# debbiemarkslab/EVcouplings

Hardware: NVIDIA H100
Metric: PLM gradient evals/s as N*L^2*q cell-ops/s (higher is better)
Workload: dtype f32 parameters/accumulation; tensor-core products as bf16 hi+lo pairs (16 mantissa bits)

## Files before the change

evcouplings_b200/csrc/plm_tc.cu:

```cuda
#include <cuda.h>
#include <cuda_bf16.h>

#include <stdlib.h>

#include <algorithm>

#include "common.cuh"
#include "internal.h"

namespace evc {

constexpr int TC_BM = 128;
constexpr int TC_BN = 192;
constexpr int TC_BK = 64;
constexpr int TC_MAX_STAGES = 8;
constexpr int TC_A_BYTES = TC_BM * TC_BK * 2;
constexpr int TC_B_BYTES = TC_BN * TC_BK * 2;
constexpr int TC_SMEM_LIMIT = 232448;
constexpr int TC_SMEM_HEAD = 2048;
constexpr int TC_THREADS = 384;
constexpr int TC_CONSUMERS = 256;
constexpr int TC_K_CHUNK = 32;
constexpr int TC_MAX_KSPLIT = 8;
constexpr int TC_REG_PRODUCER = 40;
constexpr int TC_REG_CONSUMER = 232;

__device__ __forceinline__ void mbar_wait_bounded(uint64_t *bar, uint32_t parity)
{
    uint32_t done = 0;
    for (uint64_t it = 0; it < (1ull << 31); it++) {
        asm volatile(
            "{\n.reg .pred p;\n"
            "mbarrier.try_wait.parity.shared::cta.b64 p, [%1], %2;\n"
            "selp.u32 %0, 1, 0, p;\n}\n"
            : "=r"(done)
            : "r"(smem_u32(bar)), "r"(parity)
            : "memory");
        if (done) return;
    }
    __trap();
}

__device__ __forceinline__ void mbar_arrive(uint64_t *bar)
{
    asm volatile("mbarrier.arrive.shared::cta.b64 _, [%0];" ::"r"(smem_u32(bar)) : "memory");
}

__device__ __forceinline__ void tma_load_2d(void *smem_dst, const CUtensorMap *tmap, int c0, int c1, uint64_t *bar)
{
    asm volatile(
        "cp.async.bulk.tensor.2d.shared::cluster.global.mbarrier::complete_tx::bytes [%0], [%1, {%3, %4}], [%2];"
        ::"r"(smem_u32(smem_dst)), "l"(reinterpret_cast<uint64_t>(tmap)), "r"(smem_u32(bar)), "r"(c0), "r"(c1)
        : "memory");
}

__device__ __forceinline__ void tma_load_2d_hint(void *smem_dst, const CUtensorMap *tmap, int c0, int c1,
                                                 uint64_t *bar, uint64_t policy)
{
    asm volatile(
        "cp.async.bulk.tensor.2d.shared::cluster.global.mbarrier::complete_tx::bytes.L2::cache_hint "
        "[%0], [%1, {%3, %4}], [%2], %5;"
        ::"r"(smem_u32(smem_dst)), "l"(reinterpret_cast<uint64_t>(tmap)), "r"(smem_u32(bar)), "r"(c0), "r"(c1),
        "l"(policy)
        : "memory");
}
__device__ __forceinline__ uint64_t l2_policy_evict_last()
{
    uint64_t p;
    asm volatile("createpolicy.fractional.L2::evict_last.b64 %0, 1.0;" : "=l"(p));
    return p;
}

template <int N>
__device__ __forceinline__ void setmaxnreg_dec() { asm volatile("setmaxnreg.dec.sync.aligned.u32 %0;\n" ::"n"(N)); }
template <int N>
__device__ __forceinline__ void setmaxnreg_inc() { asm volatile("setmaxnreg.inc.sync.aligned.u32 %0;\n" ::"n"(N)); }

__device__ __forceinline__ void wgmma_fence() { asm volatile("wgmma.fence.sync.aligned;" ::: "memory"); }
__device__ __forceinline__ void wgmma_commit() { asm volatile("wgmma.commit_group.sync.aligned;" ::: "memory"); }
template <int N>
__device__ __forceinline__ void wgmma_wait() { asm volatile("wgmma.wait_group.sync.aligned %0;" ::"n"(N) : "memory"); }

template <int R>
__device__ __forceinline__ void fence_regs(float *d)
{
#pragma unroll
    for (int i = 0; i < R; i++) asm volatile("" : "+f"(d[i])::"memory");
}

__device__ __forceinline__ void consumer_sync() { asm volatile("bar.sync 1, %0;" ::"n"(TC_CONSUMERS) : "memory"); }

__device__ __forceinline__ uint64_t make_desc_sw128(const void *smem_ptr)
{
    const uint32_t addr = smem_u32(smem_ptr);
    uint64_t d = 0;
    d |= (uint64_t)((addr >> 4) & 0x3FFF);
    d |= (uint64_t)1 << 16;
    d |= (uint64_t)(1024 >> 4) << 32;
    d |= (uint64_t)1 << 62;
    return d;
}

template <int N>
__device__ __forceinline__ void wgmma_bf16(float *d, uint64_t da, uint64_t db, uint32_t scale_d);
template <>
__device__ __forceinline__ void wgmma_bf16<192>(float *d, uint64_t da, uint64_t db, uint32_t scale_d)
{
    asm volatile(
        "{\n.reg .pred p;\n"
        "setp.ne.b32 p, %98, 0;\n"
        "wgmma.mma_async.sync.aligned.m64n192k16.f32.bf16.bf16 "
        "{"
        "%0, %1, %2, %3, %4, %5, %6, %7, %8, %9, %10, %11, %12, %13, %14, %15, "
        "%16, %17, %18, %19, %20, %21, %22, %23, %24, %25, %26, %27, %28, %29, %30, %31, "
        "%32, %33, %34, %35, %36, %37, %38, %39, %40, %41, %42, %43, %44, %45, %46, %47, "
        "%48, %49, %50, %51, %52, %53, %54, %55, %56, %57, %58, %59, %60, %61, %62, %63, "
        "%64, %65, %66, %67, %68, %69, %70, %71, %72, %73, %74, %75, %76, %77, %78, %79, "
        "%80, %81, %82, %83, %84, %85, %86, %87, %88, %89, %90, %91, %92, %93, %94, %95"
        "}, %96, %97, p, 1, 1, 0, 0;\n}\n"
        : "+f"(d[0]), "+f"(d[1]), "+f"(d[2]), "+f"(d[3]), "+f"(d[4]), "+f"(d[5]), "+f"(d[6]), "+f"(d[7]),
          "+f"(d[8]), "+f"(d[9]), "+f"(d[10]), "+f"(d[11]), "+f"(d[12]), "+f"(d[13]), "+f"(d[14]), "+f"(d[15]),
          "+f"(d[16]), "+f"(d[17]), "+f"(d[18]), "+f"(d[19]), "+f"(d[20]), "+f"(d[21]), "+f"(d[22]), "+f"(d[23]),
          "+f"(d[24]), "+f"(d[25]), "+f"(d[26]), "+f"(d[27]), "+f"(d[28]), "+f"(d[29]), "+f"(d[30]), "+f"(d[31]),
          "+f"(d[32]), "+f"(d[33]), "+f"(d[34]), "+f"(d[35]), "+f"(d[36]), "+f"(d[37]), "+f"(d[38]), "+f"(d[39]),
          "+f"(d[40]), "+f"(d[41]), "+f"(d[42]), "+f"(d[43]), "+f"(d[44]), "+f"(d[45]), "+f"(d[46]), "+f"(d[47]),
          "+f"(d[48]), "+f"(d[49]), "+f"(d[50]), "+f"(d[51]), "+f"(d[52]), "+f"(d[53]), "+f"(d[54]), "+f"(d[55]),
          "+f"(d[56]), "+f"(d[57]), "+f"(d[58]), "+f"(d[59]), "+f"(d[60]), "+f"(d[61]), "+f"(d[62]), "+f"(d[63]),
          "+f"(d[64]), "+f"(d[65]), "+f"(d[66]), "+f"(d[67]), "+f"(d[68]), "+f"(d[69]), "+f"(d[70]), "+f"(d[71]),
          "+f"(d[72]), "+f"(d[73]), "+f"(d[74]), "+f"(d[75]), "+f"(d[76]), "+f"(d[77]), "+f"(d[78]), "+f"(d[79]),
          "+f"(d[80]), "+f"(d[81]), "+f"(d[82]), "+f"(d[83]), "+f"(d[84]), "+f"(d[85]), "+f"(d[86]), "+f"(d[87]),
          "+f"(d[88]), "+f"(d[89]), "+f"(d[90]), "+f"(d[91]), "+f"(d[92]), "+f"(d[93]), "+f"(d[94]), "+f"(d[95])
        : "l"(da), "l"(db), "r"(scale_d));
}
template <>
__device__ __forceinline__ void wgmma_bf16<176>(float *d, uint64_t da, uint64_t db, uint32_t scale_d)
{
    asm volatile(
        "{\n.reg .pred p;\n"
        "setp.ne.b32 p, %90, 0;\n"
        "wgmma.mma_async.sync.aligned.m64n176k16.f32.bf16.bf16 "
        "{"
        "%0, %1, %2, %3, %4, %5, %6, %7, %8, %9, %10, %11, %12, %13, %14, %15, "
        "%16, %17, %18, %19, %20, %21, %22, %23, %24, %25, %26, %27, %28, %29, %30, %31, "
        "%32, %33, %34, %35, %36, %37, %38, %39, %40, %41, %42, %43, %44, %45, %46, %47, "
        "%48, %49, %50, %51, %52, %53, %54, %55, %56, %57, %58, %59, %60, %61, %62, %63, "
        "%64, %65, %66, %67, %68, %69, %70, %71, %72, %73, %74, %75, %76, %77, %78, %79, "
        "%80, %81, %82, %83, %84, %85, %86, %87"
        "}, %88, %89, p, 1, 1, 0, 0;\n}\n"
        : "+f"(d[0]), "+f"(d[1]), "+f"(d[2]), "+f"(d[3]), "+f"(d[4]), "+f"(d[5]), "+f"(d[6]), "+f"(d[7]),
          "+f"(d[8]), "+f"(d[9]), "+f"(d[10]), "+f"(d[11]), "+f"(d[12]), "+f"(d[13]), "+f"(d[14]), "+f"(d[15]),
          "+f"(d[16]), "+f"(d[17]), "+f"(d[18]), "+f"(d[19]), "+f"(d[20]), "+f"(d[21]), "+f"(d[22]), "+f"(d[23]),
          "+f"(d[24]), "+f"(d[25]), "+f"(d[26]), "+f"(d[27]), "+f"(d[28]), "+f"(d[29]), "+f"(d[30]), "+f"(d[31]),
          "+f"(d[32]), "+f"(d[33]), "+f"(d[34]), "+f"(d[35]), "+f"(d[36]), "+f"(d[37]), "+f"(d[38]), "+f"(d[39]),
          "+f"(d[40]), "+f"(d[41]), "+f"(d[42]), "+f"(d[43]), "+f"(d[44]), "+f"(d[45]), "+f"(d[46]), "+f"(d[47]),
          "+f"(d[48]), "+f"(d[49]), "+f"(d[50]), "+f"(d[51]), "+f"(d[52]), "+f"(d[53]), "+f"(d[54]), "+f"(d[55]),
          "+f"(d[56]), "+f"(d[57]), "+f"(d[58]), "+f"(d[59]), "+f"(d[60]), "+f"(d[61]), "+f"(d[62]), "+f"(d[63]),
          "+f"(d[64]), "+f"(d[65]), "+f"(d[66]), "+f"(d[67]), "+f"(d[68]), "+f"(d[69]), "+f"(d[70]), "+f"(d[71]),
          "+f"(d[72]), "+f"(d[73]), "+f"(d[74]), "+f"(d[75]), "+f"(d[76]), "+f"(d[77]), "+f"(d[78]), "+f"(d[79]),
          "+f"(d[80]), "+f"(d[81]), "+f"(d[82]), "+f"(d[83]), "+f"(d[84]), "+f"(d[85]), "+f"(d[86]), "+f"(d[87])
        : "l"(da), "l"(db), "r"(scale_d));
}

template <int N>
__device__ __forceinline__ void wgmma_kblock(float *acc, uint64_t a, uint64_t b, uint64_t a2, uint64_t b2, bool two,
                                             bool overwrite)
{
#pragma unroll
    for (int k = 0; k < TC_BK / 16; k++) {
        const uint64_t koff = (uint64_t)((k * 16 * 2) >> 4);
        wgmma_bf16<N>(acc, a + koff, b + koff, (overwrite && k == 0) ? 0u : 1u);
        if (two) wgmma_bf16<N>(acc, a2 + koff, b2 + koff, 1u);
    }
}

template <int N>
__device__ __forceinline__ void tc_mainloop(float *acc, uint64_t *full, uint64_t *empty, int &s, uint32_t &ph,
                                            int n_stages, int stage_bytes, int kb0, int kb1, uint64_t desc0,
                                            uint64_t off_a, uint64_t off_b, uint64_t off_a2, uint64_t off_b2, bool two)
{
    int prev = -1;
    for (int kb = kb0; kb < kb1; kb++) {
        mbar_wait_bounded(&full[s], ph);
        wgmma_fence();
        const uint64_t d = desc0 + (uint64_t)((s * stage_bytes) >> 4);
        wgmma_kblock<N>(acc, d + off_a, d + off_b, d + off_a2, d + off_b2, two, kb == kb0);
        wgmma_commit();
        wgmma_wait<1>();
        if (prev >= 0) mbar_arrive(&empty[prev]);
        prev = s;
        if (++s == n_stages) { s = 0; ph ^= 1u; }
    }
    wgmma_wait<0>();
    fence_regs<N / 2>(acc);
    if (prev >= 0) mbar_arrive(&empty[prev]);
}

__device__ __forceinline__ void decode_tile(int tile, int m_tiles, int n_tiles, int mgroup, int &m_tile, int &n_tile)
{
    const int full = (m_tiles / mgroup) * mgroup * n_tiles;
    if (tile < full) {
        const int per = mgroup * n_tiles;
        const int g = tile / per, r = tile - g * per;
        n_tile = r / mgroup;
        m_tile = g * mgroup + (r - n_tile * mgroup);
    } else {
        const int rem = m_tiles % mgroup, r = tile - full;
        n_tile = r / rem;
        m_tile = (m_tiles / mgroup) * mgroup + (r - n_tile * rem);
    }
}

struct TcSmem {
    uint64_t *full, *empty;
    unsigned char *ring;
};
__device__ __forceinline__ TcSmem tc_smem_layout(unsigned char *smem_dyn)
{
    unsigned char *base = reinterpret_cast<unsigned char *>((reinterpret_cast<uintptr_t>(smem_dyn) + 1023) &
                                                            ~static_cast<uintptr_t>(1023));
    TcSmem l;
    l.full = reinterpret_cast<uint64_t *>(base);
    l.empty = l.full + TC_MAX_STAGES;
    l.ring = base + 1024;
    return l;
}
__device__ __forceinline__ void tc_init_barriers(const TcSmem &l, int n_stages)
{
    if (threadIdx.x == 0) {
        for (int s = 0; s < n_stages; s++) {
            mbar_init(&l.full[s], 1);
            mbar_init(&l.empty[s], TC_CONSUMERS);
        }
        mbar_fence_init();
    }
    __syncthreads();
}

template <int SPLIT_A, int SINGLE, int ACC = 0>
__global__ void __launch_bounds__(TC_THREADS, 1)
tc_gemm_kernel(const __grid_constant__ CUtensorMap tm0, const __grid_constant__ CUtensorMap tm1,
               const __grid_constant__ CUtensorMap tm2, float *__restrict__ D, int64_t ldd, int m_tiles, int n_tiles,
               int num_kb, int k_chunk, int mgroup, int n_stages, int ksplit, int64_t plane, int acc_planes)
{
    constexpr int BYTES0 = TC_A_BYTES;
    constexpr int BYTES1 = TC_B_BYTES;
    constexpr int BYTES2 = SPLIT_A ? TC_A_BYTES : TC_B_BYTES;
    constexpr int stage_bytes = BYTES0 + BYTES1 + (SINGLE ? 0 : BYTES2);
    extern __shared__ unsigned char smem_dyn[];
    const TcSmem l = tc_smem_layout(smem_dyn);
    const int tiles = m_tiles * n_tiles;
    const int slice = (int)blockIdx.x / tiles;
    int m_tile, n_tile;
    decode_tile((int)blockIdx.x - slice * tiles, m_tiles, n_tiles, mgroup, m_tile, n_tile);
    const int kb_per = (num_kb + ksplit - 1) / ksplit;
    const int kb_begin = slice * kb_per, kb_end = min(num_kb, kb_begin + kb_per);
    tc_init_barriers(l, n_stages);

    if (threadIdx.x < 128) {
        setmaxnreg_dec<TC_REG_PRODUCER>();
        if (threadIdx.x == 0) {
            const uint64_t keep = l2_policy_evict_last();
            int s = 0;
            uint32_t ph = 0;
            for (int kb = kb_begin; kb < kb_end; kb++) {
                mbar_wait_bounded(&l.empty[s], ph ^ 1u);
                unsigned char *st = l.ring + s * stage_bytes;
                mbar_expect_tx(&l.full[s], (uint32_t)stage_bytes);
                if (SPLIT_A) {
                    tma_load_2d_hint(st, &tm0, kb * TC_BK, m_tile * TC_BM, &l.full[s], keep);
                    tma_load_2d(st + BYTES0, &tm2, kb * TC_BK, n_tile * TC_BN, &l.full[s]);
                    if (!SINGLE) tma_load_2d_hint(st + BYTES0 + BYTES1, &tm1, kb * TC_BK, m_tile * TC_BM, &l.full[s], keep);
                } else {
                    tma_load_2d(st, &tm0, kb * TC_BK, m_tile * TC_BM, &l.full[s]);
                    tma_load_2d(st + BYTES0, &tm1, kb * TC_BK, n_tile * TC_BN, &l.full[s]);
                    if (!SINGLE) tma_load_2d(st + BYTES0 + BYTES1, &tm2, kb * TC_BK, n_tile * TC_BN, &l.full[s]);
                }
                if (++s == n_stages) { s = 0; ph ^= 1u; }
            }
        }
    } else {
        setmaxnreg_inc<TC_REG_CONSUMER>();
        const int cw = (threadIdx.x >> 7) - 1;
        constexpr uint64_t OFF1 = (uint64_t)(BYTES0 >> 4), OFF2 = (uint64_t)((BYTES0 + BYTES1) >> 4);
        const uint64_t arow = (uint64_t)((cw * 64 * TC_BK * 2) >> 4);
        const uint64_t desc0 = make_desc_sw128(l.ring);
        float acc[TC_BN / 2], sum[TC_BN / 2];
#pragma unroll
        for (int u = 0; u < TC_BN / 2; u++) acc[u] = 0.f;
        const int n_chunks = (kb_end - kb_begin + k_chunk - 1) / k_chunk;
        int s = 0;
        uint32_t ph = 0;
        for (int c = 0; c < n_chunks; c++) {
            const int kb0 = kb_begin + c * k_chunk, kb1 = min(kb_end, kb0 + k_chunk);
            if (SPLIT_A) tc_mainloop<TC_BN>(acc, l.full, l.empty, s, ph, n_stages, stage_bytes, kb0, kb1, desc0,
                                            arow, OFF1, OFF2 + arow, OFF1, !SINGLE);
            else tc_mainloop<TC_BN>(acc, l.full, l.empty, s, ph, n_stages, stage_bytes, kb0, kb1, desc0,
                                    arow, OFF1, arow, OFF2, !SINGLE);
#pragma unroll
            for (int u = 0; u < TC_BN / 2; u++) sum[u] = (c == 0) ? acc[u] : sum[u] + acc[u];
        }
        const int t = threadIdx.x & 127;
        const int64_t row = (int64_t)m_tile * TC_BM + cw * 64 + (t >> 5) * 16 + ((t & 31) >> 2);
        float *out = D + slice * plane + row * ldd + (int64_t)n_tile * TC_BN + 2 * (t & 3);
        if (ACC && slice < acc_planes) {
#pragma unroll
            for (int c8 = 0; c8 < TC_BN / 8; c8++) {
                float2 *p0 = reinterpret_cast<float2 *>(out + 8 * c8);
                float2 *p1 = reinterpret_cast<float2 *>(out + 8 * ldd + 8 * c8);
                const float2 v0 = __ldcs(p0), v1 = __ldcs(p1);
                __stcs(p0, make_float2(v0.x + sum[4 * c8], v0.y + sum[4 * c8 + 1]));
                __stcs(p1, make_float2(v1.x + sum[4 * c8 + 2], v1.y + sum[4 * c8 + 3]));
            }
            return;
        }
#pragma unroll
        for (int c8 = 0; c8 < TC_BN / 8; c8++) {
            __stcs(reinterpret_cast<float2 *>(out + 8 * c8), make_float2(sum[4 * c8], sum[4 * c8 + 1]));
            __stcs(reinterpret_cast<float2 *>(out + 8 * ldd + 8 * c8), make_float2(sum[4 * c8 + 2], sum[4 * c8 + 3]));
        }
    }
}

constexpr int TF_BN = 176;
constexpr int TF_SITES = 8;
constexpr int TF_B_BYTES = TF_BN * TC_BK * 2;
constexpr int TF_PITCH = TF_BN + 1;

template <int SINGLE>
__global__ void __launch_bounds__(TC_THREADS, 1)
tc_fwd_fused_kernel(const __grid_constant__ CUtensorMap tm_x, const __grid_constant__ CUtensorMap tm_whi,
                    const __grid_constant__ CUtensorMap tm_wlo, const float *__restrict__ h,
                    const uint32_t *__restrict__ msa4, const float *__restrict__ wts,
                    __nv_bfloat16 *__restrict__ Rt_hi, __nv_bfloat16 *__restrict__ Rt_lo, int64_t Kp,
                    float *__restrict__ gh_part, double *__restrict__ fx_part, PlmGeom g, int m_tiles, int n_tiles,
                    int num_kb, int n_stages)
{
    constexpr int Q = 21;
    extern __shared__ unsigned char smem_dyn[];
    const TcSmem l = tc_smem_layout(smem_dyn);
    constexpr int stage_bytes = TC_A_BYTES + TF_B_BYTES + (SINGLE ? 0 : TF_B_BYTES);
    const int n_tile = blockIdx.x % n_tiles, m_tile = blockIdx.x / n_tiles;
    const int q = g.q;
    tc_init_barriers(l, n_stages);

    if (threadIdx.x < 128) {
        setmaxnreg_dec<TC_REG_PRODUCER>();
        if (threadIdx.x == 0) {
            const uint64_t keep = l2_policy_evict_last();
            int s = 0;
            uint32_t ph = 0;
            for (int kb = 0; kb < num_kb; kb++) {
                mbar_wait_bounded(&l.empty[s], ph ^ 1u);
                unsigned char *st = l.ring + s * stage_bytes;
                mbar_expect_tx(&l.full[s], (uint32_t)stage_bytes);
                tma_load_2d(st, &tm_x, kb * TC_BK, m_tile * TC_BM, &l.full[s]);
                tma_load_2d_hint(st + TC_A_BYTES, &tm_whi, kb * TC_BK, n_tile * TF_BN, &l.full[s], keep);
                if (!SINGLE)
                    tma_load_2d_hint(st + TC_A_BYTES + TF_B_BYTES, &tm_wlo, kb * TC_BK, n_tile * TF_BN, &l.full[s], keep);
                if (++s == n_stages) { s = 0; ph ^= 1u; }
            }
        }
        return;
    }
    setmaxnreg_inc<TC_REG_CONSUMER>();
    const int ct = threadIdx.x - 128;
    {
        const int cw = ct >> 7;
        const uint64_t arow = (uint64_t)((cw * 64 * TC_BK * 2) >> 4);
        constexpr uint64_t OFFH = (uint64_t)(TC_A_BYTES >> 4), OFFL = (uint64_t)((TC_A_BYTES + TF_B_BYTES) >> 4);
        float acc[TF_BN / 2];
#pragma unroll
        for (int u = 0; u < TF_BN / 2; u++) acc[u] = 0.f;
        int s = 0;
        uint32_t ph = 0;
        tc_mainloop<TF_BN>(acc, l.full, l.empty, s, ph, n_stages, stage_bytes, 0, num_kb, make_desc_sw128(l.ring),
                           arow, OFFH, arow, OFFL, !SINGLE);
        consumer_sync();
        float *stg = reinterpret_cast<float *>(l.ring);
        const int t = ct & 127;
        const int r0 = cw * 64 + (t >> 5) * 16 + ((t & 31) >> 2);
#pragma unroll
        for (int c8 = 0; c8 < TF_BN / 8; c8++) {
            const int col = 8 * c8 + 2 * (t & 3);
            stg[r0 * TF_PITCH + col] = acc[4 * c8];
            stg[r0 * TF_PITCH + col + 1] = acc[4 * c8 + 1];
            stg[(r0 + 8) * TF_PITCH + col] = acc[4 * c8 + 2];
            stg[(r0 + 8) * TF_PITCH + col + 1] = acc[4 * c8 + 3];
        }
        consumer_sync();
    }
    const float *stg = reinterpret_cast<const float *>(l.ring);
    const int ehalf = ct >> 7;
    const int r = ct & 127;
    const int quad = r >> 5, lane = r & 31;
    const int ntile_part = m_tiles * 4;
    const int64_t n = (int64_t)m_tile * TC_BM + r;
    const int64_t nc = n < g.N ? n : g.N - 1;
    const float wn = n < g.N ? wts[nc] : 0.f;
    const float *v = stg + r * TF_PITCH + ehalf * 88;
#pragma unroll
    for (int s = 0; s < 4; s++) {
        const int i = n_tile * TF_SITES + ehalf * 4 + s;
        if (i >= g.L) break;
        const int si = (int)((msa4[(int64_t)(i >> 2) * g.Nld + nc] >> (8 * (i & 3))) & 0xffu);
        const float w = si < q ? wn : 0.f;
        float z[Q];
        float mx = -INFINITY;
#pragma unroll
        for (int a = 0; a < Q; a++) {
            z[a] = (a < q) ? v[s * Q + a] + h[i * q + a] : -INFINITY;
            mx = fmaxf(mx, z[a]);
        }
        float zs = 0.f, sum = 0.f;
#pragma unroll
        for (int a = 0; a < Q; a++) {
            if (a == si) zs = z[a];
            z[a] = (a < q) ? expf(z[a] - mx) : 0.f;
            sum += z[a];
        }
        const double fx_local = (w == 0.f) ? 0.0 : -((double)w * (double)(zs - mx - logf(sum)));
        const float inv = w / sum;
        float *ghp = gh_part + ((int64_t)i * ntile_part + m_tile * 4 + quad) * g.S;
#pragma unroll
        for (int a = 0; a < Q; a++) {
            const float rr = z[a] * inv - (a == si ? w : 0.f);
            if (a < q) {
                if (n < g.N) {
                    const int64_t off = ((int64_t)i * q + a) * Kp + n;
                    const __nv_bfloat16 hi = __float2bfloat16_rn(rr);
                    Rt_hi[off] = hi;
                    if (!SINGLE) Rt_lo[off] = __float2bfloat16_rn(rr - __bfloat162float(hi));
                }
            }
            const float tot = warp_sum(rr);
            if (lane == 0) ghp[a] = (a < q) ? tot : 0.f;
        }
        const double fw = warp_sum(fx_local);
        if (lane == 0) fx_part[(int64_t)i * ntile_part + m_tile * 4 + quad] = fw;
    }
}

constexpr int EXP_SITES = 4;
constexpr int EXP_THREADS = 256;

template <bool PADDED>
__device__ __forceinline__ int64_t expand_row(int i, int a, int q)
{
    if (PADDED) return (int64_t)(i / TF_SITES) * TF_BN + ((i % TF_SITES) / 4) * 88 + (i % 4) * 21 + a;
    return (int64_t)i * q + a;
}

__device__ __forceinline__ void cp_async4(void *smem_dst, const void *gmem_src)
{
    asm volatile("cp.async.ca.shared.global [%0], [%1], 4;" ::"r"(smem_u32(smem_dst)), "l"(gmem_src) : "memory");
}
__device__ __forceinline__ void cp_async_wait_all() { asm volatile("cp.async.wait_all;" ::: "memory"); }

template <bool PADDED>
__global__ void __launch_bounds__(EXP_THREADS)
expand_tc_kernel(const float *__restrict__ x, __nv_bfloat16 *__restrict__ W_hi, __nv_bfloat16 *__restrict__ W_lo,
                 int L, int q, int64_t ldw, int single)
{
    __shared__ float sJ[EXP_SITES * EXP_SITES * 21 * 21];
    const int ti = blockIdx.y, tj = blockIdx.x;
    if (tj < ti) return;
    const int i0 = ti * EXP_SITES, j0 = tj * EXP_SITES;
    const int ni = min(EXP_SITES, L - i0), nj = min(EXP_SITES, L - j0);
    const int qq = q * q;
    for (int ii = 0; ii < ni; ii++) {
        const int i = i0 + ii, jlo = max(j0, i + 1);
        if (jlo >= j0 + nj) continue;
        const float *src = x + (int64_t)L * q + ((int64_t)i * (2 * L - i - 1) / 2 + (jlo - i - 1)) * qq;
        float *dst = sJ + (ii * EXP_SITES + (jlo - j0)) * qq;
        const int n = (j0 + nj - jlo) * qq;
        for (int e = threadIdx.x; e < n; e += blockDim.x) cp_async4(dst + e, src + e);
    }
    cp_async_wait_all();
    __syncthreads();
    const int lane = threadIdx.x & 31, warp = threadIdx.x >> 5;
    auto write_tile = [&](int r0, int nr, int c0, int nc) {
        const int width = nc * q;
        int csite[4], colN[4], colT[4];
#pragma unroll
        for (int k = 0; k < 4; k++) {
            const int c = 2 * lane + 64 * (k >> 1) + (k & 1);
            const int cs = c / q, cb = c - cs * q;
            csite[k] = c0 + cs;
            colN[k] = cs * qq + cb;
            colT[k] = cs * EXP_SITES * qq + cb * q;
        }
        for (int rr = warp; rr < nr * q; rr += EXP_THREADS / 32) {
            const int rs = rr / q, ra = rr - rs * q, r = r0 + rs;
            const int rowN = rs * EXP_SITES * qq + ra * q, rowT = rs * qq + ra;
            const int64_t off = expand_row<PADDED>(r, ra, q) * ldw + (int64_t)c0 * q;
            auto elem = [&](int k) -> float {
                if (r < csite[k]) return sJ[rowN + colN[k]];
                if (r > csite[k]) return sJ[rowT + colT[k]];
                return 0.f;
            };
#pragma unroll
            for (int h = 0; h < 2; h++) {
                const int c = 2 * lane + 64 * h;
                if (c >= width) continue;
                const float v0 = elem(2 * h);
                const __nv_bfloat16 h0 = __float2bfloat16_rn(v0);
                const __nv_bfloat16 l0 = __float2bfloat16_rn(v0 - __bfloat162float(h0));
                if (c + 1 < width) {
                    const float v1 = elem(2 * h + 1);
                    const __nv_bfloat16 h1 = __float2bfloat16_rn(v1);
                    const __nv_bfloat16 l1 = __float2bfloat16_rn(v1 - __bfloat162float(h1));
                    *reinterpret_cast<__nv_bfloat162 *>(W_hi + off + c) = __halves2bfloat162(h0, h1);
                    if (!single) *reinterpret_cast<__nv_bfloat162 *>(W_lo + off + c) = __halves2bfloat162(l0, l1);
                } else {
                    W_hi[off + c] = h0;
                    if (!single) W_lo[off + c] = l0;
                }
            }
        }
    };
    write_tile(i0, ni, j0, nj);
    if (ti != tj) write_tile(j0, nj, i0, ni);
}

__global__ void build_x_kernel(const uint32_t *__restrict__ msa4, __nv_bfloat16 *__restrict__ X, int64_t n0,
                               int64_t nreal, int64_t Nld, int L, int q, int64_t ldx)
{
    const int64_t r = blockIdx.x;
    const bool real = r < nreal;
    for (int e = threadIdx.x; e < L * q; e += blockDim.x) {
        const int j = e / q, b = e - j * q;
        const int code = real ? (int)((msa4[(int64_t)(j >> 2) * Nld + n0 + r] >> (8 * (j & 3))) & 0xffu) : 255;
        X[r * ldx + e] = __float2bfloat16(code == b ? 1.0f : 0.0f);
    }
}

template <int Q, bool ONEHOT>
__global__ void __launch_bounds__(128)
plm_softmax_kernel(const float *__restrict__ Zt, int64_t ldz, const float *__restrict__ h,
                   const uint32_t *__restrict__ msa4, const float *__restrict__ wts,
                   __nv_bfloat16 *__restrict__ Rt_hi, __nv_bfloat16 *__restrict__ Rt_lo, int64_t Kp,
                   float *__restrict__ gh_part, double *__restrict__ fx_part, PlmGeom g, int ntiles, int64_t n_base)
{
    __shared__ float s_gh[4 * 32];
    __shared__ double s_fx[4];
    const int tile = (int)(n_base >> 8) + blockIdx.x, i = blockIdx.y;
    const int tid = threadIdx.x, lane = tid & 31, warp = tid >> 5;
    const int64_t N = g.N;
    const int64_t nl = (int64_t)blockIdx.x * 256 + 2 * tid;
    const int64_t n0 = n_base + nl;
    const int64_t m0 = n0 < N ? n0 : ((N - 1) & ~(int64_t)1);
    const int64_t ml = m0 - n_base;
    const uint2 wi = *reinterpret_cast<const uint2 *>(msa4 + (int64_t)(i >> 2) * g.Nld + m0);
    const int sh = 8 * (i & 3);
    const int si[2] = {(int)((wi.x >> sh) & 0xffu), (int)((wi.y >> sh) & 0xffu)};
    float w[2];
    w[0] = (n0 < N && si[0] < Q) ? wts[n0] : 0.f;
    w[1] = (n0 + 1 < N && si[1] < Q) ? wts[n0 + 1] : 0.f;
    float z[2][Q];
    double fx_local = 0.0;
    if (ONEHOT) {
#pragma unroll
        for (int k = 0; k < 2; k++)
#pragma unroll
            for (int a = 0; a < Q; a++) z[k][a] = (a == si[k]) ? w[k] : 0.f;
    } else {
        float mx[2] = {-INFINITY, -INFINITY};
#pragma unroll
        for (int a = 0; a < Q; a++) {
            const float2 v = *reinterpret_cast<const float2 *>(Zt + ((int64_t)i * Q + a) * ldz + ml);
            const float ha = h[i * Q + a];
            z[0][a] = v.x + ha;
            z[1][a] = v.y + ha;
            mx[0] = fmaxf(mx[0], z[0][a]);
            mx[1] = fmaxf(mx[1], z[1][a]);
        }
#pragma unroll
        for (int k = 0; k < 2; k++) {
            float zs = 0.f, sum = 0.f;
#pragma unroll
            for (int a = 0; a < Q; a++) {
                if (a == si[k]) zs = z[k][a];
                z[k][a] = expf(z[k][a] - mx[k]);
                sum += z[k][a];
            }
            if (w[k] != 0.f) fx_local -= (double)w[k] * (double)(zs - mx[k] - logf(sum));
            const float inv = w[k] / sum;
#pragma unroll
            for (int a = 0; a < Q; a++) z[k][a] = z[k][a] * inv - (a == si[k] ? w[k] : 0.f);
        }
    }
#pragma unroll
    for (int a = 0; a < Q; a++) {
        if (n0 < N) {
            const int64_t off = ((int64_t)i * Q + a) * Kp + nl;
            const __nv_bfloat162 hi = __floats2bfloat162_rn(z[0][a], z[1][a]);
            *reinterpret_cast<__nv_bfloat162 *>(Rt_hi + off) = hi;
            if (Rt_lo != nullptr)
                *reinterpret_cast<__nv_bfloat162 *>(Rt_lo + off) =
                    __floats2bfloat162_rn(z[0][a] - __low2float(hi), z[1][a] - __high2float(hi));
        }
        const float v = warp_sum(z[0][a] + z[1][a]);
        if (lane == 0) s_gh[warp * 32 + a] = v;
    }
    const double fw = warp_sum(fx_local);
    if (lane == 0) s_fx[warp] = fw;
    __syncthreads();
    if (tid < g.S) {
        float tot = 0.f;
        if (tid < Q)
            for (int ww = 0; ww < 4; ww++) tot += s_gh[ww * 32 + tid];
        gh_part[((int64_t)i * ntiles + tile) * g.S + tid] = tot;
    }
    if (tid == 0) fx_part[(int64_t)i * ntiles + tile] = (s_fx[0] + s_fx[1]) + (s_fx[2] + s_fx[3]);
}

__global__ void build_xt_kernel(const uint32_t *__restrict__ msa4, __nv_bfloat16 *__restrict__ Xt, int64_t n0,
                                int64_t N, int64_t Nld, int64_t Kp, int L, int q)
{
    const int64_t n = (int64_t)blockIdx.x * blockDim.x + threadIdx.x;
    const int j = blockIdx.y;
    if (n >= Kp) return;
    int code = 255;
    if (n0 + n < N) code = (int)((msa4[(int64_t)(j >> 2) * Nld + n0 + n] >> (8 * (j & 3))) & 0xffu);
    for (int b = 0; b < q; b++)
        Xt[((int64_t)j * q + b) * Kp + n] = __float2bfloat16(code == b ? 1.0f : 0.0f);
}

constexpr int FIN_SITES = 4;
constexpr int FIN_W = FIN_SITES * 21;
constexpr int FIN_PITCH = FIN_W + 1;
constexpr int FIN_THREADS = 256;
constexpr int FIN_SMEM = 2 * FIN_W * FIN_PITCH * (int)sizeof(float);
constexpr int FIN_BATCH = 8;

__global__ void __launch_bounds__(FIN_THREADS)
finalize_pairs_tc_kernel(const float *__restrict__ Gd, int planes, int64_t plane, float *__restrict__ gJ, int L,
                         int q, int Np, float scale)
{
    extern __shared__ float fin_smem[];
    float *sA = fin_smem;
    float *sB = fin_smem + FIN_W * FIN_PITCH;
    const int ti = blockIdx.y, tj = blockIdx.x;
    if (tj < ti) return;
    const int i0 = ti * FIN_SITES, j0 = tj * FIN_SITES;
    const int wi = min(FIN_SITES, L - i0) * q, wj = min(FIN_SITES, L - j0) * q;
    auto stage = [&](float *dst, int row0, int rows, int col0, int cols) {
        const int V = (cols % 4 == 0) ? 4 : 1;
        const int nv = cols / V;
        const int dr = FIN_THREADS / nv, dc = FIN_THREADS - dr * nv;
        int r = threadIdx.x / nv, c = threadIdx.x - r * nv;
        while (r < rows) {
            float4 v[FIN_BATCH];
            int off[FIN_BATCH];
#pragma unroll
            for (int u = 0; u < FIN_BATCH; u++) {
                off[u] = r < rows ? r * FIN_PITCH + c * V : -1;
                if (r < rows) {
                    const float *p = Gd + (int64_t)(row0 + r) * Np + (col0 + c * V);
                    v[u] = V == 4 ? *reinterpret_cast<const float4 *>(p) : make_float4(p[0], 0.f, 0.f, 0.f);
#pragma unroll
                    for (int s = 1; s < TC_MAX_KSPLIT; s++) {
                        if (s >= planes) break;
                        const float *ps = p + s * plane;
                        const float4 w = V == 4 ? *reinterpret_cast<const float4 *>(ps) : make_float4(ps[0], 0.f, 0.f, 0.f);
                        v[u].x += w.x; v[u].y += w.y; v[u].z += w.z; v[u].w += w.w;
                    }
                }
                c += dc; r += dr;
                if (c >= nv) { c -= nv; r++; }
            }
#pragma unroll
            for (int u = 0; u < FIN_BATCH; u++) {
                if (off[u] < 0) break;
                float *d = dst + off[u];
                d[0] = v[u].x;
                if (V == 4) { d[1] = v[u].y; d[2] = v[u].z; d[3] = v[u].w; }
            }
        }
    };
    stage(sA, i0 * q, wi, j0 * q, wj);
    stage(sB, j0 * q, wj, i0 * q, wi);
    __syncthreads();
    const int qq = q * q;
    const int sj = FIN_THREADS / qq, sa = (FIN_THREADS % qq) / q, sb = FIN_THREADS % q;
    for (int ii = 0; ii * q < wi; ii++) {
        const int i = i0 + ii, jlo = max(j0, i + 1);
        const int n = (j0 + wj / q - jlo) * qq;
        if (n <= 0) continue;
        float *out = gJ + ((int64_t)i * (2 * L - i - 1) / 2 + (jlo - i - 1)) * qq;
        int jj = jlo - j0 + threadIdx.x / qq, a = (threadIdx.x % qq) / q, b = threadIdx.x % q;
        for (int e = threadIdx.x; e < n; e += FIN_THREADS) {
            const float v1 = sB[(jj * q + b) * FIN_PITCH + ii * q + a];
            const float v2 = sA[(ii * q + a) * FIN_PITCH + jj * q + b];
            out[e] = scale * (v1 + v2);
            b += sb; a += sa; jj += sj;
            if (b >= q) { b -= q; a++; }
            if (a >= q) { a -= q; jj++; }
        }
    }
}

static int env_int_once(const char *name, int *cache)
{
    if (*cache == -2) {
        const char *e = getenv(name);
        *cache = e ? atoi(e) : -1;
    }
    return *cache;
}

static int stages_for(int stage_bytes)
{
    return std::max(2, std::min(TC_MAX_STAGES, (TC_SMEM_LIMIT - TC_SMEM_HEAD) / stage_bytes));
}

typedef CUresult (*PFN_encodeTiled)(CUtensorMap *, CUtensorMapDataType, cuuint32_t, void *, const cuuint64_t *,
                                    const cuuint64_t *, const cuuint32_t *, const cuuint32_t *, CUtensorMapInterleave,
                                    CUtensorMapSwizzle, CUtensorMapL2promotion, CUtensorMapFloatOOBfill);

static PFN_encodeTiled get_encode_fn()
{
    static PFN_encodeTiled fn = nullptr;
    if (fn) return fn;
    void *p = nullptr;
    cudaDriverEntryPointQueryResult qres;
    if (cudaGetDriverEntryPoint("cuTensorMapEncodeTiled", &p, cudaEnableDefault, &qres) != cudaSuccess ||
        qres != cudaDriverEntryPointSuccess || !p)
        return nullptr;
    fn = reinterpret_cast<PFN_encodeTiled>(p);
    return fn;
}

static int make_map(CUtensorMap *m, void *base, int64_t rows, int64_t kp, int box_rows)
{
    PFN_encodeTiled fn = get_encode_fn();
    if (!fn) { set_error("cuTensorMapEncodeTiled entry point not available"); return 1; }
    cuuint64_t gdim[2] = {(cuuint64_t)kp, (cuuint64_t)rows};
    cuuint64_t gstride[1] = {(cuuint64_t)kp * 2};
    cuuint32_t box[2] = {(cuuint32_t)TC_BK, (cuuint32_t)box_rows};
    cuuint32_t estr[2] = {1, 1};
    CUresult r = fn(m, CU_TENSOR_MAP_DATA_TYPE_BFLOAT16, 2, base, gdim, gstride, box, estr,
                    CU_TENSOR_MAP_INTERLEAVE_NONE, CU_TENSOR_MAP_SWIZZLE_128B, CU_TENSOR_MAP_L2_PROMOTION_L2_256B,
                    CU_TENSOR_MAP_FLOAT_OOB_FILL_NONE);
    if (r != CUDA_SUCCESS) { set_error("cuTensorMapEncodeTiled failed with code " + std::to_string((int)r)); return 1; }
    return 0;
}

static int backward_ksplit(int64_t tiles, int num_kb, int sm_count)
{
    static int ks_env = -2;
    const int e = env_int_once("EVC_KSPLIT", &ks_env);
    int ks = 1;
    if (e > 0) {
        ks = std::min(e, TC_MAX_KSPLIT);
    } else {
        double best = 0.0;
        for (int s = 1; s <= 4 && s <= num_kb; s++) {
            const int64_t units = tiles * s;
            const double eff = (double)units / ((double)sm_count * (double)ceil_div(units, sm_count));
            if (eff >= 0.97) { ks = s; break; }
            if (eff > best) { best = eff; ks = s; }
        }
    }
    ks = std::max(1, std::min(ks, num_kb));
    return (int)ceil_div(num_kb, ceil_div(num_kb, ks));
}

int64_t plm_seq_chunk_round(int64_t seq_chunk) { return seq_chunk <= 0 ? 0 : round_up(seq_chunk, PLM_SEQ_CHUNK_ALIGN); }

void plm_tc_geometry(const PlmGeom &g, int sm_count, int64_t seq_chunk, PlmTcGeom &t)
{
    const int64_t lq = (int64_t)g.L * g.q;
    const int64_t c = plm_seq_chunk_round(seq_chunk);
    t.C = (c == 0 || c >= g.N) ? g.N : c;
    t.n_chunks = (int)ceil_div(g.N, t.C);
    t.Mp = round_up(lq, TC_BM);
    t.Np = round_up(lq, TC_BN);
    t.Kp = round_up(t.C, TC_BK);
    const int64_t tiles = (t.Mp / TC_BM) * (t.Np / TC_BN);
    t.ksplit = backward_ksplit(tiles, (int)(t.Kp / TC_BK), sm_count);
    t.ksplit_last = backward_ksplit(tiles, (int)(t.kp_chunk(t.n_chunks - 1, g.N) / TC_BK), sm_count);
    t.planes = std::max(t.ksplit, t.ksplit_last);
}

int plm_tc_build_xt(const PlmGeom &g, const PlmTcGeom &t, const uint32_t *d_msa4, void *d_xt, int64_t n0,
                    cudaStream_t st)
{
    dim3 grid((unsigned)ceil_div(t.Kp, 256), (unsigned)g.L);
    build_xt_kernel<<<grid, 256, 0, st>>>(d_msa4, reinterpret_cast<__nv_bfloat16 *>(d_xt), n0, g.N, g.Nld, t.Kp,
                                          g.L, g.q);
    EVC_KERNEL_CHECK();
    return 0;
}

int plm_tc_make_maps(const PlmTcGeom &t, void *d_xt, void *d_rt_hi, void *d_rt_lo, void *maps_out)
{
    CUtensorMap *m = reinterpret_cast<CUtensorMap *>(maps_out);
    if (make_map(&m[0], d_xt, t.Mp, t.Kp, TC_BM)) return 1;
    if (make_map(&m[1], d_rt_hi, t.Np, t.Kp, TC_BN)) return 1;
    if (make_map(&m[2], d_rt_lo, t.Np, t.Kp, TC_BN)) return 1;
    return 0;
}

int plm_tc_backward(const PlmGeom &g, const PlmTcGeom &t, const void *maps, float *d_Gd, int single, int chunk,
                    cudaStream_t st)
{
    const CUtensorMap *m = reinterpret_cast<const CUtensorMap *>(maps);
    const int stage = TC_A_BYTES + TC_B_BYTES + (single ? 0 : TC_B_BYTES);
    const int n_stages = stages_for(stage);
    const size_t smem = (size_t)n_stages * stage + TC_SMEM_HEAD;
    static int kc_env = -2;
    const int kc = env_int_once("EVC_KCHUNK", &kc_env);
    const int k_chunk = kc > 0 ? kc : TC_K_CHUNK;
    const int m_tiles = (int)(t.Mp / TC_BM), n_tiles = (int)(t.Np / TC_BN);
    const bool last = chunk == t.n_chunks - 1;
    const int ksplit = last ? t.ksplit_last : t.ksplit;
    const int num_kb = (int)(t.kp_chunk(chunk, g.N) / TC_BK);
    const int grid = m_tiles * n_tiles * ksplit;
    const int64_t plane = t.Mp * t.Np;
    if (chunk == 0) {
        if (single) {
            EVC_CUDA(cudaFuncSetAttribute(tc_gemm_kernel<0, 1>, cudaFuncAttributeMaxDynamicSharedMemorySize, TC_SMEM_LIMIT));
            tc_gemm_kernel<0, 1><<<grid, TC_THREADS, smem, st>>>(m[0], m[1], m[2], d_Gd, t.Np, m_tiles, n_tiles,
                                                                num_kb, k_chunk, m_tiles, n_stages, ksplit, plane, 0);
        } else {
            EVC_CUDA(cudaFuncSetAttribute(tc_gemm_kernel<0, 0>, cudaFuncAttributeMaxDynamicSharedMemorySize, TC_SMEM_LIMIT));
            tc_gemm_kernel<0, 0><<<grid, TC_THREADS, smem, st>>>(m[0], m[1], m[2], d_Gd, t.Np, m_tiles, n_tiles,
                                                                num_kb, k_chunk, m_tiles, n_stages, ksplit, plane, 0);
        }
    } else {
        const int acc_planes = t.ksplit;
        if (single) {
            EVC_CUDA(cudaFuncSetAttribute(tc_gemm_kernel<0, 1, 1>, cudaFuncAttributeMaxDynamicSharedMemorySize, TC_SMEM_LIMIT));
            tc_gemm_kernel<0, 1, 1><<<grid, TC_THREADS, smem, st>>>(m[0], m[1], m[2], d_Gd, t.Np, m_tiles, n_tiles,
                                                                   num_kb, k_chunk, m_tiles, n_stages, ksplit, plane,
                                                                   acc_planes);
        } else {
            EVC_CUDA(cudaFuncSetAttribute(tc_gemm_kernel<0, 0, 1>, cudaFuncAttributeMaxDynamicSharedMemorySize, TC_SMEM_LIMIT));
            tc_gemm_kernel<0, 0, 1><<<grid, TC_THREADS, smem, st>>>(m[0], m[1], m[2], d_Gd, t.Np, m_tiles, n_tiles,
                                                                   num_kb, k_chunk, m_tiles, n_stages, ksplit, plane,
                                                                   acc_planes);
        }
    }
    EVC_KERNEL_CHECK();
    return 0;
}

int plm_tc_finalize_pairs(const PlmGeom &g, const PlmTcGeom &t, const float *d_Gd, int planes, float *d_gJ,
                          float scale, cudaStream_t st)
{
    const unsigned nt = (unsigned)ceil_div(g.L, FIN_SITES);
    EVC_CUDA(cudaFuncSetAttribute(finalize_pairs_tc_kernel, cudaFuncAttributeMaxDynamicSharedMemorySize, FIN_SMEM));
    finalize_pairs_tc_kernel<<<dim3(nt, nt), FIN_THREADS, FIN_SMEM, st>>>(d_Gd, planes, t.Mp * t.Np, d_gJ, g.L, g.q,
                                                                         (int)t.Np, scale);
    EVC_KERNEL_CHECK();
    return 0;
}

void plm_tcf_geometry(const PlmGeom &g, const PlmTcGeom &tc, PlmTcfGeom &t)
{
    const int64_t lq = (int64_t)g.L * g.q;
    t.Mp = round_up(lq, TC_BM);
    t.Kw = round_up(lq, TC_BK);
    t.Ns = round_up(tc.C, TC_BN);
    t.Xrows = round_up(tc.C, 384);
    t.ntiles_s = (int)ceil_div(g.N, 256);
}

int plm_tcf_build_x(const PlmGeom &g, const PlmTcfGeom &t, const uint32_t *d_msa4, void *d_x1h, int64_t n0,
                    cudaStream_t st)
{
    build_x_kernel<<<(unsigned)t.Xrows, 256, 0, st>>>(d_msa4, reinterpret_cast<__nv_bfloat16 *>(d_x1h), n0,
                                                    std::min(t.Xrows, g.N - n0), g.Nld, g.L, g.q, t.Kw);
    EVC_KERNEL_CHECK();
    return 0;
}

int plm_tcf_make_maps(const PlmTcfGeom &t, void *d_wt_hi, void *d_wt_lo, void *d_x1h, void *maps_out)
{
    CUtensorMap *m = reinterpret_cast<CUtensorMap *>(maps_out);
    if (make_map(&m[0], d_wt_hi, t.Mp, t.Kw, TC_BM)) return 1;
    if (make_map(&m[1], d_wt_lo, t.Mp, t.Kw, TC_BM)) return 1;
    if (make_map(&m[2], d_x1h, t.Xrows, t.Kw, TC_BN)) return 1;
    return 0;
}

int plm_tcf_expand(const PlmGeom &g, const PlmTcfGeom &t, const float *d_x, void *d_wt_hi, void *d_wt_lo,
                   int single, cudaStream_t st)
{
    const unsigned nt = (unsigned)ceil_div(g.L, EXP_SITES);
    expand_tc_kernel<false><<<dim3(nt, nt), EXP_THREADS, 0, st>>>(d_x, reinterpret_cast<__nv_bfloat16 *>(d_wt_hi),
                                                                  reinterpret_cast<__nv_bfloat16 *>(d_wt_lo), g.L, g.q,
                                                                  t.Kw, single);
    EVC_KERNEL_CHECK();
    return 0;
}

static int forward_mgroup(const PlmTcfGeom &t, int single, int m_tiles)
{
    static int mg_env = -2;
    const int e = env_int_once("EVC_MGROUP", &mg_env);
    if (e > 0) return std::min(e, m_tiles);
    static int mb_env = -2;
    const int mb = env_int_once("EVC_MGROUP_MB", &mb_env);
    const double budget = (mb > 0 ? mb : 24) * 1.0e6;
    const double per_tile = (double)TC_BM * (double)t.Kw * 2.0 * (single ? 1.0 : 2.0);
    return std::max(1, std::min(m_tiles, (int)(budget / per_tile)));
}

int plm_tcf_logits(const PlmGeom &g, const PlmTcfGeom &t, const void *maps, float *d_zt, int single, int64_t nreal,
                   cudaStream_t st)
{
    const CUtensorMap *m = reinterpret_cast<const CUtensorMap *>(maps);
    const int stage = TC_A_BYTES + TC_B_BYTES + (single ? 0 : TC_A_BYTES);
    const int n_stages = stages_for(stage);
    const size_t smem = (size_t)n_stages * stage + TC_SMEM_HEAD;
    const int m_tiles = (int)(t.Mp / TC_BM), n_tiles = (int)ceil_div(nreal, TC_BN);
    const int num_kb = (int)(t.Kw / TC_BK);
    const int grid = m_tiles * n_tiles;
    const int kchunk = num_kb <= 128 ? num_kb : TC_K_CHUNK;
    const int mgroup = forward_mgroup(t, single, m_tiles);
    if (single) {
        EVC_CUDA(cudaFuncSetAttribute(tc_gemm_kernel<1, 1>, cudaFuncAttributeMaxDynamicSharedMemorySize, TC_SMEM_LIMIT));
        tc_gemm_kernel<1, 1><<<grid, TC_THREADS, smem, st>>>(m[0], m[1], m[2], d_zt, t.Ns, m_tiles, n_tiles, num_kb,
                                                            kchunk, mgroup, n_stages, 1, 0, 0);
    } else {
        EVC_CUDA(cudaFuncSetAttribute(tc_gemm_kernel<1, 0>, cudaFuncAttributeMaxDynamicSharedMemorySize, TC_SMEM_LIMIT));
        tc_gemm_kernel<1, 0><<<grid, TC_THREADS, smem, st>>>(m[0], m[1], m[2], d_zt, t.Ns, m_tiles, n_tiles, num_kb,
                                                            kchunk, mgroup, n_stages, 1, 0, 0);
    }
    EVC_KERNEL_CHECK();
    return 0;
}

template <bool ONEHOT>
static int launch_softmax(const PlmGeom &g, int ntiles, const float *d_zt, int64_t ldz, const float *d_x,
                          const uint32_t *d_msa4, const float *d_wts, __nv_bfloat16 *hi, __nv_bfloat16 *lo,
                          int64_t Kp, float *d_gh_part, double *d_fx_part, int64_t n0, int64_t nreal, cudaStream_t st)
{
    dim3 grid((unsigned)ceil_div(nreal, 256), (unsigned)g.L);
    switch (g.q) {
        case 21: plm_softmax_kernel<21, ONEHOT><<<grid, 128, 0, st>>>(d_zt, ldz, d_x, d_msa4, d_wts, hi, lo, Kp, d_gh_part, d_fx_part, g, ntiles, n0); break;
        case 20: plm_softmax_kernel<20, ONEHOT><<<grid, 128, 0, st>>>(d_zt, ldz, d_x, d_msa4, d_wts, hi, lo, Kp, d_gh_part, d_fx_part, g, ntiles, n0); break;
        case 5: plm_softmax_kernel<5, ONEHOT><<<grid, 128, 0, st>>>(d_zt, ldz, d_x, d_msa4, d_wts, hi, lo, Kp, d_gh_part, d_fx_part, g, ntiles, n0); break;
        case 4: plm_softmax_kernel<4, ONEHOT><<<grid, 128, 0, st>>>(d_zt, ldz, d_x, d_msa4, d_wts, hi, lo, Kp, d_gh_part, d_fx_part, g, ntiles, n0); break;
        default: set_error("plm softmax kernel: unsupported q"); return 1;
    }
    EVC_KERNEL_CHECK();
    return 0;
}

int plm_tcf_softmax(const PlmGeom &g, const PlmTcfGeom &t, const float *d_zt, const float *d_x,
                    const uint32_t *d_msa4, const float *d_wts, void *d_rt_hi, void *d_rt_lo, int64_t Kp,
                    float *d_gh_part, double *d_fx_part, int64_t n0, int64_t nreal, cudaStream_t st)
{
    return launch_softmax<false>(g, t.ntiles_s, d_zt, t.Ns, d_x, d_msa4, d_wts,
                                 reinterpret_cast<__nv_bfloat16 *>(d_rt_hi), reinterpret_cast<__nv_bfloat16 *>(d_rt_lo),
                                 Kp, d_gh_part, d_fx_part, n0, nreal, st);
}

int plm_tc_onehot_residual(const PlmGeom &g, int ntiles, const uint32_t *d_msa4, const float *d_wts, void *d_rt_hi,
                           void *d_rt_lo, int64_t Kp, float *d_gh_part, double *d_fx_part, int64_t n0, int64_t nreal,
                           cudaStream_t st)
{
    return launch_softmax<true>(g, ntiles, nullptr, 0, nullptr, d_msa4, d_wts,
                                reinterpret_cast<__nv_bfloat16 *>(d_rt_hi), reinterpret_cast<__nv_bfloat16 *>(d_rt_lo),
                                Kp, d_gh_part, d_fx_part, n0, nreal, st);
}

void plm_tcff_geometry(const PlmGeom &g, PlmTcffGeom &t)
{
    t.n_tiles = (int)ceil_div(g.L, TF_SITES);
    t.Np = (int64_t)t.n_tiles * TF_BN;
    t.Kw = round_up((int64_t)g.L * g.q, TC_BK);
    t.m_tiles = (int)ceil_div(g.N, TC_BM);
    t.Xrows = round_up(g.N, 384);
    t.ntile_part = t.m_tiles * 4;
}

bool plm_tcff_supported(const PlmGeom &g) { return g.S == 21; }

int plm_tcff_make_maps(const PlmTcffGeom &t, void *d_x1h, void *d_wp_hi, void *d_wp_lo, void *maps_out)
{
    CUtensorMap *m = reinterpret_cast<CUtensorMap *>(maps_out);
    if (make_map(&m[0], d_x1h, t.Xrows, t.Kw, TC_BM)) return 1;
    if (make_map(&m[1], d_wp_hi, t.Np, t.Kw, TF_BN)) return 1;
    if (make_map(&m[2], d_wp_lo, t.Np, t.Kw, TF_BN)) return 1;
    return 0;
}

int plm_tcff_expand(const PlmGeom &g, const PlmTcffGeom &t, const float *d_x, void *d_wp_hi, void *d_wp_lo,
                    int single, cudaStream_t st)
{
    const unsigned nt = (unsigned)ceil_div(g.L, EXP_SITES);
    expand_tc_kernel<true><<<dim3(nt, nt), EXP_THREADS, 0, st>>>(d_x, reinterpret_cast<__nv_bfloat16 *>(d_wp_hi),
                                                                 reinterpret_cast<__nv_bfloat16 *>(d_wp_lo), g.L, g.q,
                                                                 t.Kw, single);
    EVC_KERNEL_CHECK();
    return 0;
}

int plm_tcff_forward(const PlmGeom &g, const PlmTcffGeom &t, const void *maps, const float *d_x,
                     const uint32_t *d_msa4, const float *d_wts, void *d_rt_hi, void *d_rt_lo, int64_t Kp,
                     float *d_gh_part, double *d_fx_part, int single, cudaStream_t st)
{
    const CUtensorMap *m = reinterpret_cast<const CUtensorMap *>(maps);
    const int stage = TC_A_BYTES + TF_B_BYTES + (single ? 0 : TF_B_BYTES);
    const int n_stages = stages_for(stage);
    const size_t smem = (size_t)n_stages * stage + TC_SMEM_HEAD;
    const int grid = t.m_tiles * t.n_tiles;
    auto kernel = single ? tc_fwd_fused_kernel<1> : tc_fwd_fused_kernel<0>;
    EVC_CUDA(cudaFuncSetAttribute(kernel, cudaFuncAttributeMaxDynamicSharedMemorySize, TC_SMEM_LIMIT));
    kernel<<<grid, TC_THREADS, smem, st>>>(m[0], m[1], m[2], d_x, d_msa4, d_wts, reinterpret_cast<__nv_bfloat16 *>(d_rt_hi),
                                           reinterpret_cast<__nv_bfloat16 *>(d_rt_lo), Kp, d_gh_part, d_fx_part, g,
                                           t.m_tiles, t.n_tiles, (int)(t.Kw / TC_BK), n_stages);
    EVC_KERNEL_CHECK();
    return 0;
}

size_t plm_tc_map_bytes() { return 3 * sizeof(CUtensorMap); }

}
```

Baseline: 4561 billion.

## Make tensor-core GEMM kernel persistent over tiles with grid sized to SM count

Converts tc_gemm_kernel into a persistent kernel: each CTA loops over work units (tile × k-split slice) with a grid-stride, keeping the smem ring and barrier phase continuous across units. The launch grid is capped at the SM count for both the gradient GEMM and forward logits GEMM. This is meant to cut block launch and barrier-init overhead, let the producer prefetch the next tile while consumers finish the epilogue, and smooth wave quantisation. In exchange, the epilogue stores are serialized inside each CTA, and static round-robin assignment can still leave some SMs with one unit more than others.

```diff
diff --git a/evcouplings_b200/csrc/plm_tc.cu b/evcouplings_b200/csrc/plm_tc.cu
--- a/evcouplings_b200/csrc/plm_tc.cu
+++ b/evcouplings_b200/csrc/plm_tc.cu
@@ -248,12 +248,14 @@
     constexpr int stage_bytes = BYTES0 + BYTES1 + (SINGLE ? 0 : BYTES2);
     extern __shared__ unsigned char smem_dyn[];
     const TcSmem l = tc_smem_layout(smem_dyn);
-    const int tiles = m_tiles * n_tiles;
-    const int slice = (int)blockIdx.x / tiles;
-    int m_tile, n_tile;
-    decode_tile((int)blockIdx.x - slice * tiles, m_tiles, n_tiles, mgroup, m_tile, n_tile);
+    const int tiles = m_tiles * n_tiles, units = tiles * ksplit;
     const int kb_per = (num_kb + ksplit - 1) / ksplit;
-    const int kb_begin = slice * kb_per, kb_end = min(num_kb, kb_begin + kb_per);
+    auto unit = [&](int u, int &slice, int &m_tile, int &n_tile, int &kb_begin, int &kb_end) {
+        slice = u / tiles;
+        decode_tile(u - slice * tiles, m_tiles, n_tiles, mgroup, m_tile, n_tile);
+        kb_begin = slice * kb_per;
+        kb_end = min(num_kb, kb_begin + kb_per);
+    };
     tc_init_barriers(l, n_stages);
 
     if (threadIdx.x < 128) {
@@ -262,20 +264,25 @@
             const uint64_t keep = l2_policy_evict_last();
             int s = 0;
             uint32_t ph = 0;
-            for (int kb = kb_begin; kb < kb_end; kb++) {
-                mbar_wait_bounded(&l.empty[s], ph ^ 1u);
-                unsigned char *st = l.ring + s * stage_bytes;
-                mbar_expect_tx(&l.full[s], (uint32_t)stage_bytes);
-                if (SPLIT_A) {
-                    tma_load_2d_hint(st, &tm0, kb * TC_BK, m_tile * TC_BM, &l.full[s], keep);
-                    tma_load_2d(st + BYTES0, &tm2, kb * TC_BK, n_tile * TC_BN, &l.full[s]);
-                    if (!SINGLE) tma_load_2d_hint(st + BYTES0 + BYTES1, &tm1, kb * TC_BK, m_tile * TC_BM, &l.full[s], keep);
-                } else {
-                    tma_load_2d(st, &tm0, kb * TC_BK, m_tile * TC_BM, &l.full[s]);
-                    tma_load_2d(st + BYTES0, &tm1, kb * TC_BK, n_tile * TC_BN, &l.full[s]);
-                    if (!SINGLE) tma_load_2d(st + BYTES0 + BYTES1, &tm2, kb * TC_BK, n_tile * TC_BN, &l.full[s]);
+            for (int u = (int)blockIdx.x; u < units; u += (int)gridDim.x) {
+                int slice, m_tile, n_tile, kb_begin, kb_end;
+                unit(u, slice, m_tile, n_tile, kb_begin, kb_end);
+                for (int kb = kb_begin; kb < kb_end; kb++) {
+                    mbar_wait_bounded(&l.empty[s], ph ^ 1u);
+                    unsigned char *st = l.ring + s * stage_bytes;
+                    mbar_expect_tx(&l.full[s], (uint32_t)stage_bytes);
+                    if (SPLIT_A) {
+                        tma_load_2d_hint(st, &tm0, kb * TC_BK, m_tile * TC_BM, &l.full[s], keep);
+                        tma_load_2d(st + BYTES0, &tm2, kb * TC_BK, n_tile * TC_BN, &l.full[s]);
+                        if (!SINGLE)
+                            tma_load_2d_hint(st + BYTES0 + BYTES1, &tm1, kb * TC_BK, m_tile * TC_BM, &l.full[s], keep);
+                    } else {
+                        tma_load_2d(st, &tm0, kb * TC_BK, m_tile * TC_BM, &l.full[s]);
+                        tma_load_2d(st + BYTES0, &tm1, kb * TC_BK, n_tile * TC_BN, &l.full[s]);
+                        if (!SINGLE) tma_load_2d(st + BYTES0 + BYTES1, &tm2, kb * TC_BK, n_tile * TC_BN, &l.full[s]);
+                    }
+                    if (++s == n_stages) { s = 0; ph ^= 1u; }
                 }
-                if (++s == n_stages) { s = 0; ph ^= 1u; }
             }
         }
     } else {
@@ -284,39 +291,44 @@
         constexpr uint64_t OFF1 = (uint64_t)(BYTES0 >> 4), OFF2 = (uint64_t)((BYTES0 + BYTES1) >> 4);
         const uint64_t arow = (uint64_t)((cw * 64 * TC_BK * 2) >> 4);
         const uint64_t desc0 = make_desc_sw128(l.ring);
+        const int t = threadIdx.x & 127;
         float acc[TC_BN / 2], sum[TC_BN / 2];
 #pragma unroll
         for (int u = 0; u < TC_BN / 2; u++) acc[u] = 0.f;
-        const int n_chunks = (kb_end - kb_begin + k_chunk - 1) / k_chunk;
         int s = 0;
         uint32_t ph = 0;
-        for (int c = 0; c < n_chunks; c++) {
-            const int kb0 = kb_begin + c * k_chunk, kb1 = min(kb_end, kb0 + k_chunk);
-            if (SPLIT_A) tc_mainloop<TC_BN>(acc, l.full, l.empty, s, ph, n_stages, stage_bytes, kb0, kb1, desc0,
-                                            arow, OFF1, OFF2 + arow, OFF1, !SINGLE);
-            else tc_mainloop<TC_BN>(acc, l.full, l.empty, s, ph, n_stages, stage_bytes, kb0, kb1, desc0,
-                                    arow, OFF1, arow, OFF2, !SINGLE);
-#pragma unroll
-            for (int u = 0; u < TC_BN / 2; u++) sum[u] = (c == 0) ? acc[u] : sum[u] + acc[u];
-        }
-        const int t = threadIdx.x & 127;
-        const int64_t row = (int64_t)m_tile * TC_BM + cw * 64 + (t >> 5) * 16 + ((t & 31) >> 2);
-        float *out = D + slice * plane + row * ldd + (int64_t)n_tile * TC_BN + 2 * (t & 3);
-        if (ACC && slice < acc_planes) {
+        for (int u = (int)blockIdx.x; u < units; u += (int)gridDim.x) {
+            int slice, m_tile, n_tile, kb_begin, kb_end;
+            unit(u, slice, m_tile, n_tile, kb_begin, kb_end);
+            const int n_chunks = (kb_end - kb_begin + k_chunk - 1) / k_chunk;
+            for (int c = 0; c < n_chunks; c++) {
+                const int kb0 = kb_begin + c * k_chunk, kb1 = min(kb_end, kb0 + k_chunk);
+                if (SPLIT_A) tc_mainloop<TC_BN>(acc, l.full, l.empty, s, ph, n_stages, stage_bytes, kb0, kb1, desc0,
+                                                arow, OFF1, OFF2 + arow, OFF1, !SINGLE);
+                else tc_mainloop<TC_BN>(acc, l.full, l.empty, s, ph, n_stages, stage_bytes, kb0, kb1, desc0,
+                                        arow, OFF1, arow, OFF2, !SINGLE);
+#pragma unroll
+                for (int v = 0; v < TC_BN / 2; v++) sum[v] = (c == 0) ? acc[v] : sum[v] + acc[v];
+            }
+            const int64_t row = (int64_t)m_tile * TC_BM + cw * 64 + (t >> 5) * 16 + ((t & 31) >> 2);
+            float *out = D + slice * plane + row * ldd + (int64_t)n_tile * TC_BN + 2 * (t & 3);
+            if (ACC && slice < acc_planes) {
+#pragma unroll
+                for (int c8 = 0; c8 < TC_BN / 8; c8++) {
+                    float2 *p0 = reinterpret_cast<float2 *>(out + 8 * c8);
+                    float2 *p1 = reinterpret_cast<float2 *>(out + 8 * ldd + 8 * c8);
+                    const float2 v0 = __ldcs(p0), v1 = __ldcs(p1);
+                    __stcs(p0, make_float2(v0.x + sum[4 * c8], v0.y + sum[4 * c8 + 1]));
+                    __stcs(p1, make_float2(v1.x + sum[4 * c8 + 2], v1.y + sum[4 * c8 + 3]));
+                }
+                continue;
+            }
 #pragma unroll
             for (int c8 = 0; c8 < TC_BN / 8; c8++) {
-                float2 *p0 = reinterpret_cast<float2 *>(out + 8 * c8);
-                float2 *p1 = reinterpret_cast<float2 *>(out + 8 * ldd + 8 * c8);
-                const float2 v0 = __ldcs(p0), v1 = __ldcs(p1);
-                __stcs(p0, make_float2(v0.x + sum[4 * c8], v0.y + sum[4 * c8 + 1]));
-                __stcs(p1, make_float2(v1.x + sum[4 * c8 + 2], v1.y + sum[4 * c8 + 3]));
+                __stcs(reinterpret_cast<float2 *>(out + 8 * c8), make_float2(sum[4 * c8], sum[4 * c8 + 1]));
+                __stcs(reinterpret_cast<float2 *>(out + 8 * ldd + 8 * c8),
+                       make_float2(sum[4 * c8 + 2], sum[4 * c8 + 3]));
             }
-            return;
-        }
-#pragma unroll
-        for (int c8 = 0; c8 < TC_BN / 8; c8++) {
-            __stcs(reinterpret_cast<float2 *>(out + 8 * c8), make_float2(sum[4 * c8], sum[4 * c8 + 1]));
-            __stcs(reinterpret_cast<float2 *>(out + 8 * ldd + 8 * c8), make_float2(sum[4 * c8 + 2], sum[4 * c8 + 3]));
         }
     }
 }
@@ -709,6 +721,15 @@
     return *cache;
 }
 
+static int persistent_grid(int64_t units)
+{
+    int dev = 0, sms = 0;
+    if (cudaGetDevice(&dev) != cudaSuccess ||
+        cudaDeviceGetAttribute(&sms, cudaDevAttrMultiProcessorCount, dev) != cudaSuccess || sms <= 0)
+        sms = 132;
+    return (int)std::min<int64_t>(units, sms);
+}
+
 static int stages_for(int stage_bytes)
 {
     return std::max(2, std::min(TC_MAX_STAGES, (TC_SMEM_LIMIT - TC_SMEM_HEAD) / stage_bytes));
@@ -816,7 +837,7 @@
     const bool last = chunk == t.n_chunks - 1;
     const int ksplit = last ? t.ksplit_last : t.ksplit;
     const int num_kb = (int)(t.kp_chunk(chunk, g.N) / TC_BK);
-    const int grid = m_tiles * n_tiles * ksplit;
+    const int grid = persistent_grid((int64_t)m_tiles * n_tiles * ksplit);
     const int64_t plane = t.Mp * t.Np;
     if (chunk == 0) {
         if (single) {
@@ -917,7 +938,7 @@
     const size_t smem = (size_t)n_stages * stage + TC_SMEM_HEAD;
     const int m_tiles = (int)(t.Mp / TC_BM), n_tiles = (int)ceil_div(nreal, TC_BN);
     const int num_kb = (int)(t.Kw / TC_BK);
-    const int grid = m_tiles * n_tiles;
+    const int grid = persistent_grid((int64_t)m_tiles * n_tiles);
     const int kchunk = num_kb <= 128 ? num_kb : TC_K_CHUNK;
     const int mgroup = forward_mgroup(t, single, m_tiles);
     if (single) {
```

After: 4589 billion, median of 6. No clear change (+0.6%).
